# lucidrains/transfusion-pytorch

Measured on AMD Instinct MI355X. Metric: train samples/sec, dim512 d8 seq1024 text+latent, higher is better.
Workload: dtype bf16; 1 GPU; BASELINE config 2: Transfusion dim=512 depth=8 heads=8 dim_head=64 num_text_tokens=256 dim_latent=384; per-GPU batch 64 x seq 1024 (32 x [24 text tokens + (4,384) latent] per sample); step = pack + fwd + bwd + clip(0.5) + Adam(3e-4) (one GPU: no gradient exchange); global_batch=64, seq_len=1024, parallelism=dp1

## Files before the change

transfusion_pytorch_amd/csrc/attention.hip:

```cpp
#include "tfx_kernels.h"
#include "attn_asm_clobbers.inc"

namespace tfx {

constexpr int DH = 64;
constexpr int LDT = 72;

struct TileRegs { u32x4 r[2]; };
TFX_DEV void tile_gload(TileRegs& tr, const bf16* base, int ld, int row0, int nrows) {
#pragma unroll
  for (int i = 0; i < 2; i++) {
    int c = threadIdx.x + 256 * i;
    int row = min(row0 + (c >> 3), nrows - 1);
    tr.r[i] = *(const u32x4*)(base + (size_t)row * ld + (c & 7) * 8);
  }
}
TFX_DEV void tile_sstore(const TileRegs& tr, bf16* lds) {
#pragma unroll
  for (int i = 0; i < 2; i++) {
    int c = threadIdx.x + 256 * i;
    *(u32x4*)(lds + (c >> 3) * LDT + (c & 7) * 8) = tr.r[i];
  }
}
TFX_DEV bf16x8 lds_rowfrag(const bf16* lds, int r0, int ks) {
// ... 121 lines not shown
    int m = row_valid ? kve : 0;
#pragma unroll
    for (int o = 32; o > 0; o >>= 1) m = max(m, __shfl_xor(m, o, 64));
    if ((threadIdx.x & 63) == 0) kvl[threadIdx.x >> 6] = m;
    __syncthreads();
    lim = max(max(kvl[0], kvl[1]), max(kvl[2], kvl[3]));
  }
  return __builtin_amdgcn_readfirstlane(lim);
}
TFX_DEV bf16x8 pack8(const f32x16& v, int tt) {
  bf16x8 o;
#pragma unroll
  for (int e = 0; e < 8; e++) o[e] = f2bf(v[tt * 8 + e]);
  return o;
}
#define MFMA(a, b, c) __builtin_amdgcn_mfma_f32_32x32x16_bf16(a, b, c, 0, 0, 0)

TFX_DEV void wave_block_store(bf16* st, const bf16x4 (&v)[2][4], bf16* g0, int ld, int rows_valid, int lane = -1) {
  const int l = (lane >= 0 ? lane : (int)threadIdx.x) & 63, hi = l >> 5, r = l & 31, ch = l & 7;
  if (((ld & 7) | (int)(((uintptr_t)g0 >> 1) & 7)) != 0) {
    if (r < rows_valid) {
#pragma unroll
      for (int db = 0; db < 2; db++)
#pragma unroll
        for (int rg = 0; rg < 4; rg++) *(bf16x4*)(g0 + (size_t)r * ld + db * 32 + 8 * rg + 4 * hi) = v[db][rg];
    }
    return;
  }
#pragma unroll
  for (int db = 0; db < 2; db++)
#pragma unroll
    for (int rg = 0; rg < 4; rg++) {
      const int col = db * 32 + 8 * rg + 4 * hi;
      *(bf16x4*)(st + r * 64 + (((col >> 3) ^ ((r >> 1) & 7)) << 3) + (col & 7)) = v[db][rg];
    }
  bf16x8 t[4];
#pragma unroll
  for (int q = 0; q < 4; q++) {
    const int row = q * 8 + (l >> 3);
    t[q] = *(const bf16x8*)(st + row * 64 + ((ch ^ ((row >> 1) & 7)) << 3));
  }
#pragma unroll
  for (int q = 0; q < 4; q++) {
    const int row = q * 8 + (l >> 3);
    if (row < rows_valid) *(bf16x8*)(g0 + (size_t)row * ld + ch * 8) = t[q];
  }
}

template <int WHICH>
TFX_DEV void wave_block_store_nr(bf16* st, const bf16x4 (&v)[2][4], const tfx_attn_args& p, size_t tok, int colq, int rows_valid, float (&pg)[8], int lane = -1) {
  const int l = (lane >= 0 ? lane : (int)threadIdx.x) & 63, hi = l >> 5, r = l & 31, ch = l & 7;
  if (rows_valid <= 0) return;
#pragma unroll
  for (int db = 0; db < 2; db++)
#pragma unroll
    for (int rg = 0; rg < 4; rg++) {
      const int col = db * 32 + 8 * rg + 4 * hi;
      *(bf16x4*)(st + r * 64 + (((col >> 3) ^ ((r >> 1) & 7)) << 3) + (col & 7)) = v[db][rg];
    }
  if (!p.nr_gamma_q) {
    const int last = max(rows_valid - 1, 0);
    int pos[4];
#pragma unroll
    for (int q = 0; q < 4; q++) pos[q] = p.nr_rot_pos[tok + min(q * 8 + (l >> 3), last)];
#pragma unroll
    for (int q = 0; q < 4; q++) {
      const int row = q * 8 + (l >> 3), rd = min(row, last);
      const f32x4 cs = *(const f32x4*)(p.nr_cos + (size_t)pos[q] * 32 + ch * 4), sn = *(const f32x4*)(p.nr_sin + (size_t)pos[q] * 32 + ch * 4);
      const bf16x8 t = *(const bf16x8*)(st + rd * 64 + ((ch ^ ((rd >> 1) & 7)) << 3));
      const bf16x8 o = qk_rope_bwd_chunk(t, WHICH == 0 ? p.nr_q_scale : 1.f, cs, sn);
      if (row < rows_valid) *(bf16x8*)(p.nr_dqkv + (tok + row) * p.nr_ld_dqkv + colq + ch * 8) = o;
    }
    return;
  }
  const float sc = (WHICH == 0 ? p.nr_q_scale : 1.f) * (p.nr_norm_scale > 0.f ? p.nr_norm_scale : 8.f);
  const float* gmp = (WHICH == 0 ? p.nr_gamma_q : p.nr_gamma_k) + ch * 8;
  const f32x4 g0 = *(const f32x4*)gmp, g1 = *(const f32x4*)(gmp + 4);
  bf16x8 x8[4], t[4];
  f32x4 cs[4], sn[4];
  const int last = max(rows_valid - 1, 0);
#pragma unroll
  for (int q = 0; q < 4; q++) {
    const int row = min(q * 8 + (l >> 3), last);
    const size_t tt = tok + row;
    x8[q] = *(const bf16x8*)(p.nr_qkv + tt * p.nr_ld_qkv + colq + ch * 8);
    const int pos = p.nr_rot_pos[tt];
    cs[q] = *(const f32x4*)(p.nr_cos + (size_t)pos * 32 + ch * 4);
    sn[q] = *(const f32x4*)(p.nr_sin + (size_t)pos * 32 + ch * 4);
  }
#pragma unroll
  for (int q = 0; q < 4; q++) {
    const int row = min(q * 8 + (l >> 3), last);
    t[q] = *(const bf16x8*)(st + row * 64 + ((ch ^ ((row >> 1) & 7)) << 3));
  }
#pragma unroll
  for (int q = 0; q < 4; q++) {
    const int row = q * 8 + (l >> 3);
    const bool live = row < rows_valid;
    float xv[8], qq = 0.f;
#pragma unroll
    for (int e = 0; e < 8; e++) { xv[e] = bf2f(x8[q][e]); qq = fmaf(xv[e], xv[e], qq); }
    qq = group8_sum(qq);
    const float inv = qq > 1e-24f ? __builtin_amdgcn_rsqf(qq) : 1e12f;
    const float isc = live ? inv * sc : 0.f;
    float dyn[8], S = 0.f;
#pragma unroll
    for (int i = 0; i < 4; i++) {
      const float da = bf2f(t[q][2 * i]), db = bf2f(t[q][2 * i + 1]);
      const float ga = fmaf(db, sn[q][i], da * cs[q][i]);
      const float gb = fmaf(-da, sn[q][i], db * cs[q][i]);
      const float gma = i < 2 ? g0[2 * i] : g1[2 * i - 4], gmb = i < 2 ? g0[2 * i + 1] : g1[2 * i - 3];
      const float ca = sc * (1.f + gma), cb = sc * (1.f + gmb);
      const float ta = ga * xv[2 * i], tb = gb * xv[2 * i + 1];
      pg[2 * i] = fmaf(ta, isc, pg[2 * i]); pg[2 * i + 1] = fmaf(tb, isc, pg[2 * i + 1]);
      S = fmaf(ta, ca, S); S = fmaf(tb, cb, S);
      dyn[2 * i] = ga * ca; dyn[2 * i + 1] = gb * cb;
    }
    S = group8_sum(S);
    const float k = S * inv * inv * inv;
    bf16x8 o;
#pragma unroll
    for (int e = 0; e < 8; e++) o[e] = f2bf(fmaf(dyn[e], inv, -(xv[e] * k)));
    if (live) *(bf16x8*)(p.nr_dqkv + (tok + row) * p.nr_ld_dqkv + colq + ch * 8) = o;
  }
}
TFX_DEV void nr_flush_dgamma(float (&pg)[8], float* sg , float* dgamma, int t = -1) {
  const int tx = t >= 0 ? t : (int)threadIdx.x;
#pragma unroll
  for (int e = 0; e < 8; e++) {
#pragma unroll
    for (int m = 8; m < 64; m <<= 1) pg[e] += __shfl_xor(pg[e], m, 64);
  }
  const int lane = tx & 63, wv = tx >> 6;
  if (lane < 8) {
#pragma unroll
    for (int e = 0; e < 8; e++) sg[wv * 64 + lane * 8 + e] = pg[e];
  }
  __syncthreads();
  if (tx < 64) {
    const float s4 = sg[tx] + sg[64 + tx] + sg[128 + tx] + sg[192 + tx];
    if (s4 != 0.f) atomicAdd(dgamma + tx, s4);
  }
}
struct BlockId { int tile, h, b; };
TFX_DEV BlockId decode_block(int order, int ntile, bool heavy_last_tile) {
  BlockId o;
  (void)order;
  o.tile = heavy_last_tile ? ntile - 1 - (int)blockIdx.z : (int)blockIdx.z;
  o.h = blockIdx.x; o.b = blockIdx.y;
  return o;
}

#define MFMA_ACC(acc, a, b) asm volatile("v_mfma_f32_32x32x16_bf16 %0, %1, %2, %0" : "+v"(acc), "+v"(a), "+v"(b))
TFX_DEV void fwd_phase(const f32x16& s_cur, f32x16& s_nxt, u32x4 (&p_prev)[2], u32x4 (&p_cur)[2], f32x16 (&o)[2], const bf16x8 (&qf)[4],
                       const bf16* Kt_nxt, int kb_nxt, const bf16* Vt_prev, int kb_prev, float (&lsum)[2]) {
  const int hi = (threadIdx.x >> 5) & 1;
  bf16x8 frag[2];
  auto fetch = [&](int m) -> bf16x8 {
    if (m < 4) return dma_rowfrag(Kt_nxt, kb_nxt * 32, m);
    const int ra = kb_prev * 32 + 16 * ((m - 4) >> 1) + 4 * hi;
    return dma_tr8(Vt_prev, ra, ra + 8, (m & 1) * 32);
  };
  frag[0] = fetch(0);
#pragma unroll
  for (int ch = 0; ch < 8; ch++) {
    if (ch < 7) frag[(ch + 1) & 1] = fetch(ch + 1);
    float e0 = __builtin_amdgcn_exp2f(s_cur[2 * ch]), e1 = __builtin_amdgcn_exp2f(s_cur[2 * ch + 1]);
    if (ch == 0) asm volatile("v_mfma_f32_32x32x16_bf16 %0, %3, %4, 0" : "=&v"(s_nxt), "+v"(e0), "+v"(e1), "+v"(frag[0]) : "v"(qf[0]));
    else if (ch < 4) asm volatile("v_mfma_f32_32x32x16_bf16 %0, %3, %4, %0" : "+v"(s_nxt), "+v"(e0), "+v"(e1), "+v"(frag[ch & 1]) : "v"(qf[ch]));
    else asm volatile("v_mfma_f32_32x32x16_bf16 %0, %3, %4, %0" : "+v"(o[ch & 1]), "+v"(e0), "+v"(e1), "+v"(frag[ch & 1]), "+v"(p_prev[(ch - 4) >> 1]));
    lsum[0] += e0; lsum[1] += e1;
    bf16x2 pk2; pk2[0] = f2bf(e0); pk2[1] = f2bf(e1);
    uint32_t pk = __builtin_bit_cast(uint32_t, pk2);
    asm volatile("" : "+v"(lsum[0]), "+v"(lsum[1]), "+v"(pk));
    p_cur[ch >> 2][ch & 3] = pk;
    __builtin_amdgcn_sched_barrier(0);
  }
}

template <bool ROW>
TFX_DEV void fwd_phase_any(f32x16& s_cur, f32x16& s_nxt, u32x4 (&p_prev)[2], u32x4 (&p_cur)[2], f32x16 (&o)[2], const bf16x8 (&qf)[4],
                           const bf16* Kt_nxt, int kb_nxt, const bf16* Vt_prev, int kb_prev, float (&lsum)[2], const SoftCap& c, int key0, int kve,
                           bool mask, unsigned long long* ts = nullptr) {
#ifdef TFX_ATTN_TIMING
  unsigned long long t0 = __builtin_readcyclecounter();
#endif
  softcap16<ROW>(s_cur, c);
  if (mask) {
#pragma unroll
    for (int r = 0; r < 16; r++) s_cur[r] = key0 + (r & 3) + 8 * (r >> 2) < kve ? s_cur[r] : -__builtin_inff();
  }
#ifdef TFX_ATTN_TIMING
  asm volatile("" : "+v"(s_cur));
  unsigned long long t1 = __builtin_readcyclecounter();
#endif
  fwd_phase(s_cur, s_nxt, p_prev, p_cur, o, qf, Kt_nxt, kb_nxt, Vt_prev, kb_prev, lsum);
#ifdef TFX_ATTN_TIMING
  asm volatile("" : "+v"(s_nxt), "+v"(o[0]), "+v"(o[1]));
  ts[2] += t1 - t0; ts[3] += __builtin_readcyclecounter() - t1;
#endif
}

TFX_DEV void fwd_drain(u32x4 (&p_prev)[2], f32x16 (&o)[2], const bf16* Vt_prev, int kb_prev) {
  const int hi = (threadIdx.x >> 5) & 1;
  bf16x8 vt[4];
#pragma unroll
  for (int m = 0; m < 4; m++) { const int ra = kb_prev * 32 + 16 * (m >> 1) + 4 * hi; vt[m] = dma_tr8(Vt_prev, ra, ra + 8, (m & 1) * 32); }
#pragma unroll
  for (int m = 0; m < 4; m++) MFMA_ACC(o[m & 1], vt[m], p_prev[m >> 1]);
  asm volatile("s_nop 7" : "+v"(vt[0]), "+v"(vt[1]), "+v"(vt[2]), "+v"(vt[3]), "+v"(p_prev[0]), "+v"(p_prev[1]));
}

template <bool ASM, bool ROW = false>
__global__ __launch_bounds__(256, 2) void attn_fwd_pipe_kernel(tfx_attn_args p) {
  __shared__ __attribute__((aligned(1024))) bf16 Ks[3][64 * 64];
  __shared__ __attribute__((aligned(1024))) bf16 Vs[3][64 * 64];
  const int l = threadIdx.x & 63, w = threadIdx.x >> 6, hi = l >> 5;
  const BlockId bi = decode_block(p.order, (p.n + 127) / 128, true);
  const int h = bi.h, b = bi.b, q0 = bi.tile * 128;
  const int n = p.q_cnt ? p.q_cnt[b] : p.n;
  if (q0 >= n) return;
  const int nkv = p.n_kv > 0 ? p.n_kv : n;
  const size_t tok0 = p.q_row0 ? (size_t)p.q_row0[b] : (size_t)b * n, tokk = (size_t)b * nkv;
  const bf16* qb = p.q + tok0 * p.ld_q + h * DH;
  const bf16* kb_ = p.k + tokk * p.ld_k + h * DH;
  const bf16* vb = p.v + tokk * p.ld_v + h * DH;
  const int qrow = q0 + w * 32 + (l & 31);
  const int qc = min(qrow, n - 1);
  const int kve = p.kv_end[tok0 + qc];
  const int kv_limit = tile_kv_limit(p, tok0, q0, n, kve, qrow < n);
  const int nt = (kv_limit + 63) / 64;
  bf16x8 qf[4];
#pragma unroll
  for (int ks = 0; ks < 4; ks++) qf[ks] = g_rowfrag(qb, p.ld_q, qrow, n, ks);
  const SoftCap sc_ = make_softcap(p.softcap, p.sc_plan);
  const int kve_min = wave_min_i(kve);
  asm volatile("" : "+v"(qf[0]), "+v"(qf[1]), "+v"(qf[2]), "+v"(qf[3]));
  asm volatile("s_waitcnt vmcnt(0)" ::: "memory");
  tile_dma(kb_, p.ld_k, 0, nkv, Ks[0]);
  tile_dma(vb, p.ld_v, 0, nkv, Vs[0]);
  if (nt > 1) tile_dma(kb_, p.ld_k, 64, nkv, Ks[1]);

  f32x16 o[2], sA, sB;
  u32x4 pA[2], pB[2];
#pragma unroll
  for (int i = 0; i < 2; i++) {
#pragma unroll
    for (int r = 0; r < 16; r++) o[i][r] = 0.f;
#pragma unroll
    for (int e = 0; e < 4; e++) { pA[i][e] = 0u; pB[i][e] = 0u; }
  }
#pragma unroll
  for (int r = 0; r < 16; r++) { sA[r] = 0.f; sB[r] = 0.f; }
  float lsum[2] = {0.f, 0.f};
  int kslot = 0, vslot = 0;
#ifdef TFX_ATTN_TIMING
  unsigned long long tsec[4] = {0, 0, 0, 0}, tprev = __builtin_readcyclecounter();
#define AT_MARK(i) { const unsigned long long tn = __builtin_readcyclecounter(); tsec[i] += tn - tprev; tprev = tn; }
#define TS_ARG , tsec
#else
#define AT_MARK(i)
#define TS_ARG
#endif
  int j0 = 0;
  if constexpr (ASM) {
    const int kve_blk = __builtin_amdgcn_readfirstlane(p.kv_end[tok0 + q0]);
    const int nfull = __builtin_amdgcn_readfirstlane(min(kve_blk >> 6, (nkv - 128) >> 6));
    if (nfull > 0 && sc_.mode <= 1) {
      const int wu = __builtin_amdgcn_readfirstlane(w);
      const uint32_t ldsK = (uint32_t)(size_t)(lds_void_t*)&Ks[0][0], ldsV = (uint32_t)(size_t)(lds_void_t*)&Vs[0][0];
      uint32_t ka[4], vaA[2], vaB[2], dk[2], dv[2];
#pragma unroll
      for (int ks = 0; ks < 4; ks++) ka[ks] = ldsK + 2u * (uint32_t)((l & 31) * 64 + (((2 * ks + hi) ^ swz_f(l & 31)) << 3));
      {
        const int q = l & 15, ra = 4 * hi + (q >> 2), rb = ra + 8;
#pragma unroll
        for (int db = 0; db < 2; db++) {
          const int col = db * 32 + 16 * ((l >> 4) & 1) + 4 * (q & 3);
          vaA[db] = ldsV + 2u * (uint32_t)(ra * 64 + (((col >> 3) ^ swz_f(ra)) << 3) + (col & 7));
          vaB[db] = ldsV + 2u * (uint32_t)(rb * 64 + (((col >> 3) ^ swz_f(rb)) << 3) + (col & 7));
        }
      }
#pragma unroll
      for (int jp = 0; jp < 2; jp++) {
        const int r = w * 16 + jp * 8 + (l >> 3), c = (l & 7) ^ swz_f(r);
        dk[jp] = 2u * (uint32_t)(r * p.ld_k + c * 8);
        dv[jp] = 2u * (uint32_t)(r * p.ld_v + c * 8);
      }
      const uint64_t baseK = (uint64_t)(uintptr_t)kb_, baseV = (uint64_t)(uintptr_t)vb;
      u32x4 rsK, rsV;
      rsK[0] = __builtin_amdgcn_readfirstlane((uint32_t)baseK); rsK[1] = __builtin_amdgcn_readfirstlane((uint32_t)(baseK >> 32) & 0xffffu); rsK[2] = 0xffffff00u; rsK[3] = 0x00020000u;
      rsV[0] = __builtin_amdgcn_readfirstlane((uint32_t)baseV); rsV[1] = __builtin_amdgcn_readfirstlane((uint32_t)(baseV >> 32) & 0xffffu); rsV[2] = 0xffffff00u; rsV[3] = 0x00020000u;
      const uint32_t stk = __builtin_amdgcn_readfirstlane(128u * (uint32_t)p.ld_k), stv = __builtin_amdgcn_readfirstlane(128u * (uint32_t)p.ld_v);
      uint32_t sko = 2u * stk, svo = stv, cnt = (uint32_t)nfull;
      const uint32_t mk = __builtin_amdgcn_readfirstlane(ldsK + (uint32_t)wu * 2048u), mv = __builtin_amdgcn_readfirstlane(ldsV + (uint32_t)wu * 2048u);
      const float p1 = sc_.p1, p3 = sc_.p3, p5 = sc_.p5;
      u32x4 q0f = __builtin_bit_cast(u32x4, qf[0]), q1f = __builtin_bit_cast(u32x4, qf[1]), q2f = __builtin_bit_cast(u32x4, qf[2]), q3f = __builtin_bit_cast(u32x4, qf[3]);
#define AF_OPERANDS                                                                                                                                  \
          : [o0] "+&v"(o[0]), [o1] "+&v"(o[1]), "+{v[64:79]}"(sA), "+{v[104:107]}"(pB[0]), "+{v[108:111]}"(pB[1]), "+{v112}"(lsum[0]), "+{v113}"(lsum[1]),    \
            [sko] "+&s"(sko), [svo] "+&s"(svo), [cnt] "+&s"(cnt)                                                                                     \
          : [qf0] "v"(q0f), [qf1] "v"(q1f), [qf2] "v"(q2f), [qf3] "v"(q3f), [ka0] "v"(ka[0]), [ka1] "v"(ka[1]), [ka2] "v"(ka[2]), [ka3] "v"(ka[3]),  \
            [va0] "v"(vaA[0]), [va1] "v"(vaA[1]), [vb0] "v"(vaB[0]), [vb1] "v"(vaB[1]), [dk0] "v"(dk[0]), [dk1] "v"(dk[1]), [dv0] "v"(dv[0]), [dv1] "v"(dv[1]), \
            [rsk] "s"(rsK), [rsv] "s"(rsV), [stk] "s"(stk), [stv] "s"(stv), [mk] "s"(mk), [mv] "s"(mv), [p1] "v"(p1), [p3] AF_P3(p3), [p5] "s"(p5)   \
          : "memory", "scc", "v80", "v81", "v82", "v83", "v84", "v85", "v86", "v87", "v88", "v89", "v90", "v91", "v92", "v93", "v94", "v95",         \
            "v96", "v97", "v98", "v99", "v100", "v101", "v102", "v103", "v116", "v117", "v118", "v119", "v120", "v121", "v122", "v123", "v124",      \
            "v125", "v126", "v127", "v128", "v129", "v130", "v131", "v132", "v133", "v134", "v135", "v136", "v137", "v138", "v139", "v140", "v141",  \
            "v142", "v143", "v144", "v145", "v146", "v147", "v148", "v149", "v150", "v151"
      if (sc_.mode == 0) {
#define AF_P3 "s"
        asm volatile(
#include "attn_fwd_loop_m0.inc"
            AF_OPERANDS);
#undef AF_P3
      } else {
#define AF_P3 "v"
        asm volatile(
#include "attn_fwd_loop_m1.inc"
            AF_OPERANDS);
#undef AF_P3
      }
#undef AF_OPERANDS
      j0 = nfull;
      kslot = vslot = nfull % 3;
    }
  }
  for (int j = j0; j < nt; j++) {
    asm volatile("s_waitcnt vmcnt(0)" ::: "memory");
    __builtin_amdgcn_s_barrier();
    AT_MARK(0)
    const int kslot1 = kslot == 2 ? 0 : kslot + 1, kslot2 = kslot1 == 2 ? 0 : kslot1 + 1;
    const int vslot1 = vslot == 2 ? 0 : vslot + 1, vprev = vslot == 0 ? 2 : vslot - 1;
    if (j + 2 < nt) tile_dma(kb_, p.ld_k, (j + 2) * 64, nkv, Ks[kslot2]);
    if (j + 1 < nt) tile_dma(vb, p.ld_v, (j + 1) * 64, nkv, Vs[vslot1]);
    AT_MARK(1)
    if (j == 0) {
      sA = __builtin_amdgcn_mfma_f32_32x32x16_bf16(dma_rowfrag(Ks[0], 0, 0), qf[0], f32x16{}, 0, 0, 0);
#pragma unroll
      for (int ks = 1; ks < 4; ks++) sA = MFMA(dma_rowfrag(Ks[0], 0, ks), qf[ks], sA);
    }
    int u = 2 * j;
    fwd_phase_any<ROW>(sA, sB, pB, pA, o, qf, Ks[kslot], 1, j == 0 ? Vs[vslot] : Vs[vprev], 1, lsum, sc_, u * 32 + 4 * hi, kve, (u + 1) * 32 > kve_min TS_ARG);
    u = 2 * j + 1;
    fwd_phase_any<ROW>(sB, sA, pA, pB, o, qf, Ks[kslot1], 0, Vs[vslot], 0, lsum, sc_, u * 32 + 4 * hi, kve, (u + 1) * 32 > kve_min TS_ARG);
    kslot = kslot1; vslot = vslot1;
#ifdef TFX_ATTN_TIMING
    tprev = __builtin_readcyclecounter();
#endif
  }
#ifdef TFX_ATTN_TIMING
  if (l == 0) {
    unsigned long long* ob = (unsigned long long*)p.dq + ((((size_t)b * p.h + h) * ((n + 127) / 128) + bi.tile) * 4 + w) * 5;
    for (int i = 0; i < 4; i++) ob[i] = tsec[i];
    ob[4] = nt;
  }
#endif
#undef AT_MARK
#undef TS_ARG
  fwd_drain(pB, o, Vs[vslot == 0 ? 2 : vslot - 1], 1);
  asm volatile("s_nop 15\n\ts_nop 15" : "+v"(o[0]), "+v"(o[1]));
  float ls = lsum[0] + lsum[1];
  ls += __shfl_xor(ls, 32, 64);
  {
    const float g = p.gate ? sigmoidf_(bf2f(p.gate[(tok0 + qc) * p.ld_gate + h])) : 1.f;
    bf16x4 ov[2][4];
    if (p.laser) {
      const float rl = __builtin_amdgcn_rcpf(ls);
#pragma unroll
      for (int db = 0; db < 2; db++)
#pragma unroll
        for (int rg = 0; rg < 4; rg++)
#pragma unroll
          for (int e = 0; e < 4; e++) ov[db][rg][e] = f2bf(g * __logf(o[db][rg * 4 + e] * rl));
    } else {
      const float sc = g * __builtin_amdgcn_rcpf(ls);
#pragma unroll
      for (int db = 0; db < 2; db++)
#pragma unroll
        for (int rg = 0; rg < 4; rg++)
#pragma unroll
          for (int e = 0; e < 4; e++) ov[db][rg][e] = f2bf(o[db][rg * 4 + e] * sc);
    }
    __syncthreads();
    wave_block_store(&Ks[0][0] + w * 2048, ov, p.out + (tok0 + q0 + w * 32) * p.ld_out + h * DH, p.ld_out, n - (q0 + w * 32));
    if (qrow < n && hi == 0) p.lse[((size_t)b * p.h + h) * p.n + qrow] = __log2f(ls) * LN2;
  }
}

__global__ __launch_bounds__(256) void attn_bwd_prep_kernel(tfx_attn_args p) {
  const unsigned gid = blockIdx.x * blockDim.x + threadIdx.x;
  const unsigned vid = gid >> 3;
  const int sub = gid & 7;
  const unsigned T = (unsigned)p.b * p.n;
  if (vid >= T * p.h) return;
  const unsigned t = vid / (unsigned)p.h; const int h = (int)(vid - t * p.h);
  const bf16x8 d8 = *(const bf16x8*)(p.dout + (size_t)t * p.ld_dout + h * DH + sub * 8);
  const bf16x8 o8 = *(const bf16x8*)(p.out + (size_t)t * p.ld_out + h * DH + sub * 8);
  const float g = p.gate ? sigmoidf_(bf2f(p.gate[(size_t)t * p.ld_gate + h])) : 1.f;
  if (p.laser) {
    const float rg = __builtin_amdgcn_rcpf(fmaxf(g, 1e-30f));
    float dg = 0.f, ds = 0.f; bf16x8 e8;
#pragma unroll
    for (int e = 0; e < 8; e++) {
      const float d = bf2f(d8[e]), og = bf2f(o8[e]);
      dg += d * og; ds += d;
      e8[e] = f2bf(d * g * __expf(-og * rg));
    }
    *(bf16x8*)(p.do_eff + (size_t)t * p.ld_do + h * DH + sub * 8) = e8;
    dg = group8_sum(dg); ds = group8_sum(ds);
    if (sub == 0) {
      const unsigned bb = t / (unsigned)p.n, i = t - bb * p.n;
      p.delta[((size_t)bb * p.h + h) * p.n + i] = ds * g;
      if (p.gate) p.dgate[(size_t)t * p.ld_dgate + h] = f2bf(dg * (1.f - g));
    }
    return;
  }
  float dl = 0.f; bf16x8 e8;
#pragma unroll
  for (int e = 0; e < 8; e++) { float d = bf2f(d8[e]); dl += d * bf2f(o8[e]); e8[e] = f2bf(d * g); }
  *(bf16x8*)(p.do_eff + (size_t)t * p.ld_do + h * DH + sub * 8) = e8;
  dl = group8_sum(dl);
  if (sub == 0) {
    const unsigned bb = t / (unsigned)p.n, i = t - bb * p.n;
    p.delta[((size_t)bb * p.h + h) * p.n + i] = dl;
    if (p.gate) p.dgate[(size_t)t * p.ld_dgate + h] = f2bf(dl * (1.f - g));
  }
}

__global__ __launch_bounds__(256, 2) void attn_bwd_dq_kernel(tfx_attn_args p) {
  __shared__ __attribute__((aligned(16))) bf16 Ks[64 * LDT];
  __shared__ __attribute__((aligned(16))) bf16 Vs[64 * LDT];
  const int l = threadIdx.x & 63, w = threadIdx.x >> 6, hi = l >> 5;
  const int n = p.n;
  const BlockId bi = decode_block(p.order, (n + 127) / 128, true);
  const int h = bi.h, b = bi.b, q0 = bi.tile * 128;
  const size_t tok0 = (size_t)b * n;
  const bf16* qb = p.q + tok0 * p.ld_q + h * DH;
  const bf16* kb_ = p.k + tok0 * p.ld_k + h * DH;
  const bf16* vb = p.v + tok0 * p.ld_v + h * DH;
  const bf16* dob = p.do_eff + tok0 * p.ld_do + h * DH;
  const int qrow = q0 + w * 32 + (l & 31);
  const int qc = min(qrow, n - 1);
  const int kve = p.kv_end[tok0 + qc];
  const int kv_limit = p.kv_end[tok0 + min(q0 + 127, n - 1)];
  const int nt = (kv_limit + 63) / 64;
  const float lse2 = p.lse[((size_t)b * p.h + h) * n + qc] * LOG2E;
  float dlt;
  const int kve_min = wave_min_i(kve);

  bf16x8 qf[4], dof[4];
  dlt = p.delta[((size_t)b * p.h + h) * n + qc];
#pragma unroll
  for (int ks = 0; ks < 4; ks++) { qf[ks] = g_rowfrag(qb, p.ld_q, qrow, n, ks); dof[ks] = g_rowfrag(dob, p.ld_do, qrow, n, ks); }
  f32x16 dq[2];
#pragma unroll
  for (int i = 0; i < 2; i++)
#pragma unroll
    for (int r = 0; r < 16; r++) dq[i][r] = 0.f;
  const SoftCap sc_ = make_softcap(p.softcap, p.sc_plan);
  f32x16 zero16;
#pragma unroll
  for (int r = 0; r < 16; r++) zero16[r] = 0.f;
  asm volatile("" : "+v"(zero16));

  TileRegs kr, vr;
  tile_gload(kr, kb_, p.ld_k, 0, n);
  tile_gload(vr, vb, p.ld_v, 0, n);
  for (int j = 0; j < nt; j++) {
    __syncthreads();
    tile_sstore(kr, Ks); tile_sstore(vr, Vs);
    __syncthreads();
    if (j + 1 < nt) { tile_gload(kr, kb_, p.ld_k, (j + 1) * 64, n); tile_gload(vr, vb, p.ld_v, (j + 1) * 64, n); }
    const bool need_mask = (j + 1) * 64 > kve_min;
#pragma unroll
    for (int kb = 0; kb < 2; kb++) {
      f32x16 s = MFMA(lds_rowfrag(Ks, kb * 32, 0), qf[0], zero16);
      f32x16 dp = MFMA(lds_rowfrag(Vs, kb * 32, 0), dof[0], zero16);
#pragma unroll
      for (int ks = 1; ks < 4; ks++) {
        s = MFMA(lds_rowfrag(Ks, kb * 32, ks), qf[ks], s);
        dp = MFMA(lds_rowfrag(Vs, kb * 32, ks), dof[ks], dp);
      }
      if (sc_.mode == 0) {
#pragma unroll
        for (int r = 0; r < 16; r++) {
          const float u = s[r] * s[r];
          dp[r] = (dp[r] - dlt) * fmaf(u, sc_.d3, sc_.d1);
          s[r] = __builtin_amdgcn_exp2f(fmaf(s[r], fmaf(u, sc_.p3, sc_.p1), -lse2));
        }
      } else if (sc_.mode == 1) {
#pragma unroll
        for (int r = 0; r < 16; r++) {
          const float u = s[r] * s[r];
          dp[r] = (dp[r] - dlt) * fmaf(u, fmaf(u, sc_.d5, sc_.d3), sc_.d1);
          s[r] = __builtin_amdgcn_exp2f(fmaf(s[r], fmaf(u, fmaf(u, sc_.p5, sc_.p3), sc_.p1), -lse2));
        }
      } else {
        softcap16(s, sc_);
#pragma unroll
        for (int r = 0; r < 16; r++) {
          const float dth = fmaf(s[r] * s[r], -sc_.g2, 1.f);
          dp[r] = (dp[r] - dlt) * dth;
          s[r] = __builtin_amdgcn_exp2f(s[r] - lse2);
        }
      }
      if (need_mask) {
        const int key0 = j * 64 + kb * 32 + 4 * hi;
#pragma unroll
        for (int r = 0; r < 16; r++) s[r] = key0 + (r & 3) + 8 * (r >> 2) < kve ? s[r] : 0.f;
      }
#pragma unroll
      for (int r = 0; r < 16; r++) s[r] *= dp[r];
#pragma unroll
      for (int tt = 0; tt < 2; tt++) {
        const bf16x8 dsf = pack8(s, tt);
        const int ra = kb * 32 + 16 * tt + 4 * hi;
#pragma unroll
        for (int db = 0; db < 2; db++) dq[db] = MFMA(lds_tr8(Ks, LDT, ra, ra + 8, db * 32), dsf, dq[db]);
      }
    }
  }
  {
    bf16x4 ov[2][4];
#pragma unroll
    for (int db = 0; db < 2; db++)
#pragma unroll
      for (int rg = 0; rg < 4; rg++)
#pragma unroll
        for (int e = 0; e < 4; e++) ov[db][rg][e] = f2bf(dq[db][rg * 4 + e]);
    __syncthreads();
    if (p.nr_qkv) {
      __shared__ float sg[4 * 64];
      float pg[8];
#pragma unroll
      for (int e = 0; e < 8; e++) pg[e] = 0.f;
      wave_block_store_nr<0>((w < 2 ? Ks : Vs) + (w & 1) * 2048, ov, p, tok0 + q0 + w * 32, h * DH, n - (q0 + w * 32), pg);
      if (p.nr_gamma_q) nr_flush_dgamma(pg, sg, p.nr_dgamma_q);
    } else
    wave_block_store((w < 2 ? Ks : Vs) + (w & 1) * 2048, ov, p.dq + (tok0 + q0 + w * 32) * p.ld_dq + h * DH, p.ld_dq, n - (q0 + w * 32));
// ... 239 lines not shown
  for (int rg = 0; rg < 4; rg++) {
    const int ql = ql0 + 8 * rg;
    const f32x4 ls4 = *(const f32x4*)(s_lse + ql), dl4 = *(const f32x4*)(s_dlt + ql);
    const int* kv4 = s_kve + ql;
#pragma unroll
    for (int e = 0; e < 4; e++) {
      const int r = rg * 4 + e;
      const float a = s[r];
      float arg, dth;
      if constexpr (MODE == 0) {
        const float u = a * a;
        dth = fmaf(u, c.d3, c.d1);
        arg = fmaf(a, fmaf(u, c.p3, c.p1), -ls4[e]);
      } else if constexpr (MODE == 1) {
        const float u = a * a;
        dth = fmaf(u, fmaf(u, c.d5, c.d3), c.d1);
        arg = fmaf(a, fmaf(u, fmaf(u, c.p5, c.p3), c.p1), -ls4[e]);
      } else {
        dth = fmaf(a * a, -g2, 1.f);
        arg = a - ls4[e];
      }
      float pv = __builtin_amdgcn_exp2f(arg);
      if (MASK) pv = krow < kv4[e] ? pv : 0.f;
      pr[r] = pv;
      s[r] = pv * ((dp[r] - dl4[e]) * dth);
    }
  }
}

__global__ __launch_bounds__(256, 2) void attn_bwd_dkv_kernel(tfx_attn_args p) {
  __shared__ __attribute__((aligned(16))) bf16 Qs[64 * LDT];
  __shared__ __attribute__((aligned(16))) bf16 Ds[64 * LDT];
  __shared__ __attribute__((aligned(16))) float s_lse[64], s_dlt[64];
  __shared__ __attribute__((aligned(16))) int s_kve[64];
  const int l = threadIdx.x & 63, w = threadIdx.x >> 6, hi = l >> 5;
  const int n = p.n;
  const BlockId bi = decode_block(p.order, (n + 127) / 128, false);
  const int h = bi.h, b = bi.b, k0 = bi.tile * 128;
  const size_t tok0 = (size_t)b * n;
  const bf16* qb = p.q + tok0 * p.ld_q + h * DH;
  const bf16* kb_ = p.k + tok0 * p.ld_k + h * DH;
  const bf16* vb = p.v + tok0 * p.ld_v + h * DH;
  const bf16* dob = p.do_eff + tok0 * p.ld_do + h * DH;
  const float* lseb = p.lse + ((size_t)b * p.h + h) * n;
  const float* dltb = p.delta + ((size_t)b * p.h + h) * n;
  const int krow = k0 + w * 32 + (l & 31);
  const int qt0 = p.q_start[tok0 + min(k0, n - 1)] / 64;
  const int qt1 = (n + 63) / 64;

  bf16x8 kf[4], vf[4];
#pragma unroll
  for (int ks = 0; ks < 4; ks++) { kf[ks] = g_rowfrag(kb_, p.ld_k, krow, n, ks); vf[ks] = g_rowfrag(vb, p.ld_v, krow, n, ks); }
  f32x16 dk[2], dv[2];
#pragma unroll
  for (int i = 0; i < 2; i++)
#pragma unroll
    for (int r = 0; r < 16; r++) { dk[i][r] = 0.f; dv[i][r] = 0.f; }
  const SoftCap sc_ = make_softcap(p.softcap, p.sc_plan);
  const int kw_last = k0 + w * 32 + 31;

  TileRegs qr, dr;
  float st_l = 0.f, st_d = 0.f; int st_k = 0;
  auto stats_gload = [&](int jt) {
    if (threadIdx.x < 64) {
      const int qi = jt * 64 + threadIdx.x;
      const int qcl = min(qi, n - 1);
      st_l = lseb[qcl]; st_d = dltb[qcl];
      st_k = qi < n ? p.kv_end[tok0 + qcl] : 0;
    }
  };
  tile_gload(qr, qb, p.ld_q, qt0 * 64, n);
  tile_gload(dr, dob, p.ld_do, qt0 * 64, n);
  stats_gload(qt0);
  for (int jt = qt0; jt < qt1; jt++) {
    __syncthreads();
    tile_sstore(qr, Qs); tile_sstore(dr, Ds);
    if (threadIdx.x < 64) { s_lse[threadIdx.x] = st_l * LOG2E; s_dlt[threadIdx.x] = st_d; s_kve[threadIdx.x] = st_k; }
    __syncthreads();
    if (jt + 1 < qt1) { tile_gload(qr, qb, p.ld_q, (jt + 1) * 64, n); tile_gload(dr, dob, p.ld_do, (jt + 1) * 64, n); stats_gload(jt + 1); }
#pragma unroll
    for (int qb2 = 0; qb2 < 2; qb2++) {
      {
        const int lastr = min(31, n - 1 - (jt * 64 + qb2 * 32));
        if (__builtin_amdgcn_readfirstlane((int)(lastr < 0 || s_kve[qb2 * 32 + max(lastr, 0)] <= k0 + w * 32)) != 0) continue;
      }
      f32x16 s, dp;
#pragma unroll
      for (int r = 0; r < 16; r++) { s[r] = 0.f; dp[r] = 0.f; }
#pragma unroll
      for (int ks = 0; ks < 4; ks++) {
        s = MFMA(lds_rowfrag(Qs, qb2 * 32, ks), kf[ks], s);
        dp = MFMA(lds_rowfrag(Ds, qb2 * 32, ks), vf[ks], dp);
      }
      if (sc_.mode == 2) softcap16(s, sc_);
      const bool need_mask = __builtin_amdgcn_readfirstlane((int)(kw_last >= s_kve[qb2 * 32] || jt * 64 + qb2 * 32 + 31 >= n)) != 0;
      f32x16 pr;
      const int ql0 = qb2 * 32 + 4 * hi;
      if (sc_.mode == 0) {
        if (need_mask) dkv_scores<true, 0>(s, dp, pr, s_lse, s_dlt, s_kve, ql0, krow, sc_.g2, sc_);
        else dkv_scores<false, 0>(s, dp, pr, s_lse, s_dlt, s_kve, ql0, krow, sc_.g2, sc_);
      } else if (sc_.mode == 1) {
        if (need_mask) dkv_scores<true, 1>(s, dp, pr, s_lse, s_dlt, s_kve, ql0, krow, sc_.g2, sc_);
        else dkv_scores<false, 1>(s, dp, pr, s_lse, s_dlt, s_kve, ql0, krow, sc_.g2, sc_);
      } else {
        if (need_mask) dkv_scores<true, 2>(s, dp, pr, s_lse, s_dlt, s_kve, ql0, krow, sc_.g2, sc_);
        else dkv_scores<false, 2>(s, dp, pr, s_lse, s_dlt, s_kve, ql0, krow, sc_.g2, sc_);
      }
#pragma unroll
      for (int tt = 0; tt < 2; tt++) {
        const bf16x8 pf = pack8(pr, tt), dsf = pack8(s, tt);
        const int ra = qb2 * 32 + 16 * tt + 4 * hi;
#pragma unroll
        for (int db = 0; db < 2; db++) {
          dv[db] = MFMA(lds_tr8(Ds, LDT, ra, ra + 8, db * 32), pf, dv[db]);
          dk[db] = MFMA(lds_tr8(Qs, LDT, ra, ra + 8, db * 32), dsf, dk[db]);
        }
      }
    }
  }
  {
    bf16x4 kv[2][4], vv[2][4];
#pragma unroll
    for (int db = 0; db < 2; db++)
#pragma unroll
      for (int rg = 0; rg < 4; rg++)
#pragma unroll
        for (int e = 0; e < 4; e++) { kv[db][rg][e] = f2bf(dk[db][rg * 4 + e]); vv[db][rg][e] = f2bf(dv[db][rg * 4 + e]); }
    __syncthreads();
    bf16* st = (w < 2 ? Qs : Ds) + (w & 1) * 2048;
    const int rows = n - (k0 + w * 32);
    if (p.nr_qkv) {
      __shared__ float sg[4 * 64];
      float pg[8];
#pragma unroll
      for (int e = 0; e < 8; e++) pg[e] = 0.f;
      wave_block_store_nr<1>(st, kv, p, tok0 + k0 + w * 32, (p.h + h) * DH, rows, pg);
      wave_block_store(st, vv, p.dv + (tok0 + k0 + w * 32) * p.ld_dv + h * DH, p.ld_dv, rows);
      if (p.nr_gamma_q) nr_flush_dgamma(pg, sg, p.nr_dgamma_k);
    } else {
      wave_block_store(st, kv, p.dk + (tok0 + k0 + w * 32) * p.ld_dk + h * DH, p.ld_dk, rows);
      wave_block_store(st, vv, p.dv + (tok0 + k0 + w * 32) * p.ld_dv + h * DH, p.ld_dv, rows);
    }
  }
}

static dim3 attn_grid(const tfx_attn_args& q) { return dim3(q.h, q.b, (q.n + 127) / 128); }
int attn_fwd(const tfx_attn_args& p, hipStream_t s) {
  if (p.n <= 0 || p.b <= 0 || p.h <= 0) return -1;
  if ((p.ld_q | p.ld_k | p.ld_v | p.ld_out) & 7) return -2;
  if (!(p.softcap > 0.f) || p.softcap * LOG2E > 96.f) return -3;
  tfx_attn_args q = p; q.order = 1;
  static int use_asm = -1;
  if (use_asm < 0) { const char* e = getenv("TFX_ATTN_ASM"); use_asm = (e && e[0] == '1') ? 1 : 0; }
  if (use_asm && p.n_kv == 0 && !p.q_cnt && !p.q_row0 && p.sc_plan) hipLaunchKernelGGL(attn_fwd_pipe_kernel<true>, attn_grid(q), dim3(256), 0, s, q);
  else if (p.n_kv > 0 || p.q_cnt || p.q_row0) hipLaunchKernelGGL((attn_fwd_pipe_kernel<false, true>), attn_grid(q), dim3(256), 0, s, q);
  else hipLaunchKernelGGL(attn_fwd_pipe_kernel<false>, attn_grid(q), dim3(256), 0, s, q);
  return (int)hipGetLastError();
}
int attn_bwd(const tfx_attn_args& p, hipStream_t s) {
  if (p.n <= 0 || p.b <= 0 || p.h <= 0) return -1;
  if ((p.ld_q | p.ld_k | p.ld_v | p.ld_out | p.ld_dout | p.ld_do | p.ld_dq | p.ld_dk | p.ld_dv) & 7) return -2;
  if (!(p.softcap > 0.f) || p.softcap * LOG2E > 96.f) return -3;
  long long nthreads = (long long)p.b * p.n * p.h * 8;
  if (nthreads >= (1ll << 31)) return -4;
  if (p.nr_qkv) {
    if (!p.nr_dqkv || !p.nr_gamma_q != !p.nr_gamma_k || !p.nr_rot_pos || !p.nr_cos || !p.nr_sin) return -5;
    if (p.nr_gamma_q && (!p.nr_dgamma_q || !p.nr_dgamma_k)) return -5;
    if (((p.nr_ld_qkv | p.nr_ld_dqkv) & 7) || (((uintptr_t)p.nr_qkv | (uintptr_t)p.nr_dqkv) & 15)) return -5;
  }
  tfx_attn_args q = p; q.order = 1;
  static int pipe = -1;
  if (pipe < 0) { const char* e = getenv("TFX_ATTN_BWD_PIPE"); pipe = (e && e[0] == '0') ? 0 : 1; }
  hipLaunchKernelGGL(attn_bwd_prep_kernel, dim3((unsigned)((nthreads + 255) / 256)), dim3(256), 0, s, q);
  hipLaunchKernelGGL(attn_bwd_dkv_kernel, attn_grid(q), dim3(256), 0, s, q);
  if (pipe) hipLaunchKernelGGL(attn_bwd_dq_pipe_kernel, attn_grid(q), dim3(256), 0, s, q);
  else hipLaunchKernelGGL(attn_bwd_dq_kernel, attn_grid(q), dim3(256), 0, s, q);
  return (int)hipGetLastError();
}

}
```

Before: 2619 samples/s.

## Stop attention forward compute early per wave at its last needed key block

Adds a STOP variant of the forward attention kernel, on by default. Each wave computes the last 32-key chunk any of its rows can attend to and stops softmax/MFMA work there. For the remaining tiles it only takes part in barriers and DMA issue, so block-level synchronisation still holds. A half-tile tail path skips the next-S MFMAs, and a per-block hash rotates wave-to-row assignment to spread the imbalance. This cuts wasted masked work in the causal/latent-block attention pattern, at the cost of more code paths and possible correctness risk in the slot bookkeeping.

```diff
diff --git a/transfusion_pytorch_amd/csrc/attention.hip b/transfusion_pytorch_amd/csrc/attention.hip
--- a/transfusion_pytorch_amd/csrc/attention.hip
+++ b/transfusion_pytorch_amd/csrc/attention.hip
@@ -297,21 +297,26 @@
 }
 
 #define MFMA_ACC(acc, a, b) asm volatile("v_mfma_f32_32x32x16_bf16 %0, %1, %2, %0" : "+v"(acc), "+v"(a), "+v"(b))
+#ifdef TFX_ATTN_TIMING
+enum { AT_PROLOGUE = 4, AT_TILE_INT, AT_TILE_BND, AT_NTILE_INT, AT_NTILE_BND, AT_DRAIN, AT_EPI_BARRIER, AT_STORE_ISSUE, AT_STORE_ACK, AT_NT, AT_LU, AT_LIFE, AT_NSEC };
+#endif
+template <bool S_NXT = true>
 TFX_DEV void fwd_phase(const f32x16& s_cur, f32x16& s_nxt, u32x4 (&p_prev)[2], u32x4 (&p_cur)[2], f32x16 (&o)[2], const bf16x8 (&qf)[4],
-                       const bf16* Kt_nxt, int kb_nxt, const bf16* Vt_prev, int kb_prev, float (&lsum)[2]) {
-  const int hi = (threadIdx.x >> 5) & 1;
+                       const bf16* Kt_nxt, int kb_nxt, const bf16* Vt_prev, int kb_prev, float (&lsum)[2], int lane = -1) {
+  const int hi = ((lane >= 0 ? lane : (int)threadIdx.x) >> 5) & 1;
   bf16x8 frag[2];
   auto fetch = [&](int m) -> bf16x8 {
-    if (m < 4) return dma_rowfrag(Kt_nxt, kb_nxt * 32, m);
+    if (m < 4) return dma_rowfrag(Kt_nxt, kb_nxt * 32, m, lane);
     const int ra = kb_prev * 32 + 16 * ((m - 4) >> 1) + 4 * hi;
-    return dma_tr8(Vt_prev, ra, ra + 8, (m & 1) * 32);
+    return dma_tr8(Vt_prev, ra, ra + 8, (m & 1) * 32, lane);
   };
-  frag[0] = fetch(0);
+  if (S_NXT) frag[0] = fetch(0);
 #pragma unroll
   for (int ch = 0; ch < 8; ch++) {
-    if (ch < 7) frag[(ch + 1) & 1] = fetch(ch + 1);
+    if (ch < 7 && (S_NXT || ch >= 3)) frag[(ch + 1) & 1] = fetch(ch + 1);
     float e0 = __builtin_amdgcn_exp2f(s_cur[2 * ch]), e1 = __builtin_amdgcn_exp2f(s_cur[2 * ch + 1]);
-    if (ch == 0) asm volatile("v_mfma_f32_32x32x16_bf16 %0, %3, %4, 0" : "=&v"(s_nxt), "+v"(e0), "+v"(e1), "+v"(frag[0]) : "v"(qf[0]));
+    if (ch < 4 && !S_NXT) asm volatile("" : "+v"(e0), "+v"(e1));
+    else if (ch == 0) asm volatile("v_mfma_f32_32x32x16_bf16 %0, %3, %4, 0" : "=&v"(s_nxt), "+v"(e0), "+v"(e1), "+v"(frag[0]) : "v"(qf[0]));
     else if (ch < 4) asm volatile("v_mfma_f32_32x32x16_bf16 %0, %3, %4, %0" : "+v"(s_nxt), "+v"(e0), "+v"(e1), "+v"(frag[ch & 1]) : "v"(qf[ch]));
     else asm volatile("v_mfma_f32_32x32x16_bf16 %0, %3, %4, %0" : "+v"(o[ch & 1]), "+v"(e0), "+v"(e1), "+v"(frag[ch & 1]), "+v"(p_prev[(ch - 4) >> 1]));
     lsum[0] += e0; lsum[1] += e1;
@@ -323,10 +328,10 @@
   }
 }
 
-template <bool ROW>
+template <bool ROW, bool S_NXT = true>
 TFX_DEV void fwd_phase_any(f32x16& s_cur, f32x16& s_nxt, u32x4 (&p_prev)[2], u32x4 (&p_cur)[2], f32x16 (&o)[2], const bf16x8 (&qf)[4],
                            const bf16* Kt_nxt, int kb_nxt, const bf16* Vt_prev, int kb_prev, float (&lsum)[2], const SoftCap& c, int key0, int kve,
-                           bool mask, unsigned long long* ts = nullptr) {
+                           bool mask, unsigned long long* ts = nullptr, int lane = -1) {
 #ifdef TFX_ATTN_TIMING
   unsigned long long t0 = __builtin_readcyclecounter();
 #endif
@@ -339,30 +344,45 @@
   asm volatile("" : "+v"(s_cur));
   unsigned long long t1 = __builtin_readcyclecounter();
 #endif
-  fwd_phase(s_cur, s_nxt, p_prev, p_cur, o, qf, Kt_nxt, kb_nxt, Vt_prev, kb_prev, lsum);
+  fwd_phase<S_NXT>(s_cur, s_nxt, p_prev, p_cur, o, qf, Kt_nxt, kb_nxt, Vt_prev, kb_prev, lsum, lane);
 #ifdef TFX_ATTN_TIMING
   asm volatile("" : "+v"(s_nxt), "+v"(o[0]), "+v"(o[1]));
   ts[2] += t1 - t0; ts[3] += __builtin_readcyclecounter() - t1;
 #endif
 }
 
-TFX_DEV void fwd_drain(u32x4 (&p_prev)[2], f32x16 (&o)[2], const bf16* Vt_prev, int kb_prev) {
-  const int hi = (threadIdx.x >> 5) & 1;
+TFX_DEV void fwd_drain(u32x4 (&p_prev)[2], f32x16 (&o)[2], const bf16* Vt_prev, int kb_prev, int lane = -1) {
+  const int hi = ((lane >= 0 ? lane : (int)threadIdx.x) >> 5) & 1;
   bf16x8 vt[4];
 #pragma unroll
-  for (int m = 0; m < 4; m++) { const int ra = kb_prev * 32 + 16 * (m >> 1) + 4 * hi; vt[m] = dma_tr8(Vt_prev, ra, ra + 8, (m & 1) * 32); }
+  for (int m = 0; m < 4; m++) { const int ra = kb_prev * 32 + 16 * (m >> 1) + 4 * hi; vt[m] = dma_tr8(Vt_prev, ra, ra + 8, (m & 1) * 32, lane); }
 #pragma unroll
   for (int m = 0; m < 4; m++) MFMA_ACC(o[m & 1], vt[m], p_prev[m >> 1]);
   asm volatile("s_nop 7" : "+v"(vt[0]), "+v"(vt[1]), "+v"(vt[2]), "+v"(vt[3]), "+v"(p_prev[0]), "+v"(p_prev[1]));
 }
 
-template <bool ASM, bool ROW = false>
+template <bool ASM, bool ROW = false, bool STOP = false>
 __global__ __launch_bounds__(256, 2) void attn_fwd_pipe_kernel(tfx_attn_args p) {
   __shared__ __attribute__((aligned(1024))) bf16 Ks[3][64 * 64];
   __shared__ __attribute__((aligned(1024))) bf16 Vs[3][64 * 64];
-  const int l = threadIdx.x & 63, w = threadIdx.x >> 6, hi = l >> 5;
+#ifdef TFX_ATTN_TIMING
+  unsigned long long tsec[AT_NT], tprev = __builtin_readcyclecounter();
+  const unsigned long long tborn = tprev;
+#pragma unroll
+  for (int i = 0; i < AT_NT; i++) tsec[i] = 0;
+#define AT_MARK(i) { const unsigned long long tn = __builtin_readcyclecounter(); tsec[i] += tn - tprev; tprev = tn; }
+#define TS_ARG , tsec
+#define TS_ARG_L , tsec,
+#else
+#define AT_MARK(i)
+#define TS_ARG
+#define TS_ARG_L , nullptr,
+#endif
+  const int l = threadIdx.x & 63, hi = l >> 5;
   const BlockId bi = decode_block(p.order, (p.n + 127) / 128, true);
   const int h = bi.h, b = bi.b, q0 = bi.tile * 128;
+  const unsigned lin = blockIdx.x + gridDim.x * (blockIdx.y + gridDim.y * blockIdx.z);
+  const int w = STOP ? (int)((__builtin_amdgcn_readfirstlane(threadIdx.x >> 6) + (lin ^ (lin >> 2) ^ (lin >> 4) ^ (lin >> 6) ^ (lin >> 8) ^ (lin >> 10))) & 3) : (int)(threadIdx.x >> 6);
   const int n = p.q_cnt ? p.q_cnt[b] : p.n;
   if (q0 >= n) return;
   const int nkv = p.n_kv > 0 ? p.n_kv : n;
@@ -380,11 +400,13 @@
   for (int ks = 0; ks < 4; ks++) qf[ks] = g_rowfrag(qb, p.ld_q, qrow, n, ks);
   const SoftCap sc_ = make_softcap(p.softcap, p.sc_plan);
   const int kve_min = wave_min_i(kve);
+  const int lu = STOP ? min(max(wave_max_i(qrow < n ? kve : 0) - 1, 0) >> 5, 2 * nt - 1) : 2 * nt - 1;
   asm volatile("" : "+v"(qf[0]), "+v"(qf[1]), "+v"(qf[2]), "+v"(qf[3]));
   asm volatile("s_waitcnt vmcnt(0)" ::: "memory");
   tile_dma(kb_, p.ld_k, 0, nkv, Ks[0]);
   tile_dma(vb, p.ld_v, 0, nkv, Vs[0]);
   if (nt > 1) tile_dma(kb_, p.ld_k, 64, nkv, Ks[1]);
+  AT_MARK(AT_PROLOGUE)
 
   f32x16 o[2], sA, sB;
   u32x4 pA[2], pB[2];
@@ -399,14 +421,6 @@
   for (int r = 0; r < 16; r++) { sA[r] = 0.f; sB[r] = 0.f; }
   float lsum[2] = {0.f, 0.f};
   int kslot = 0, vslot = 0;
-#ifdef TFX_ATTN_TIMING
-  unsigned long long tsec[4] = {0, 0, 0, 0}, tprev = __builtin_readcyclecounter();
-#define AT_MARK(i) { const unsigned long long tn = __builtin_readcyclecounter(); tsec[i] += tn - tprev; tprev = tn; }
-#define TS_ARG , tsec
-#else
-#define AT_MARK(i)
-#define TS_ARG
-#endif
   int j0 = 0;
   if constexpr (ASM) {
     const int kve_blk = __builtin_amdgcn_readfirstlane(p.kv_end[tok0 + q0]);
@@ -469,39 +483,67 @@
       kslot = vslot = nfull % 3;
     }
   }
-  for (int j = j0; j < nt; j++) {
-    asm volatile("s_waitcnt vmcnt(0)" ::: "memory");
-    __builtin_amdgcn_s_barrier();
-    AT_MARK(0)
-    const int kslot1 = kslot == 2 ? 0 : kslot + 1, kslot2 = kslot1 == 2 ? 0 : kslot1 + 1;
-    const int vslot1 = vslot == 2 ? 0 : vslot + 1, vprev = vslot == 0 ? 2 : vslot - 1;
-    if (j + 2 < nt) tile_dma(kb_, p.ld_k, (j + 2) * 64, nkv, Ks[kslot2]);
-    if (j + 1 < nt) tile_dma(vb, p.ld_v, (j + 1) * 64, nkv, Vs[vslot1]);
-    AT_MARK(1)
-    if (j == 0) {
-      sA = __builtin_amdgcn_mfma_f32_32x32x16_bf16(dma_rowfrag(Ks[0], 0, 0), qf[0], f32x16{}, 0, 0, 0);
-#pragma unroll
-      for (int ks = 1; ks < 4; ks++) sA = MFMA(dma_rowfrag(Ks[0], 0, ks), qf[ks], sA);
-    }
+#ifdef TFX_ATTN_TIMING
+  unsigned long long ttile = tprev;
+#define AT_TILE_END(j) { const unsigned long long tn = __builtin_readcyclecounter(); const int bnd = (2 * (j) + 2) * 32 > kve_min ? 1 : 0;               \
+                         tsec[AT_TILE_INT + bnd] += tn - ttile; tsec[AT_NTILE_INT + bnd] += 1; ttile = tn; tprev = tn; }
+#else
+#define AT_TILE_END(j)
+#endif
+#define FWD_TILE_TOP(j)                                                                                                                                \
+    asm volatile("s_waitcnt vmcnt(0)" ::: "memory");                                            \
+    __builtin_amdgcn_s_barrier();                                              \
+    AT_MARK(0)                                                                                                                                         \
+    const int kslot1 = kslot == 2 ? 0 : kslot + 1, kslot2 = kslot1 == 2 ? 0 : kslot1 + 1;                                                             \
+    const int vslot1 = vslot == 2 ? 0 : vslot + 1, vprev = vslot == 0 ? 2 : vslot - 1;                                                                \
+    if ((j) + 2 < nt) tile_dma(kb_, p.ld_k, ((j) + 2) * 64, nkv, Ks[kslot2]);                                                                         \
+    if ((j) + 1 < nt) tile_dma(vb, p.ld_v, ((j) + 1) * 64, nkv, Vs[vslot1]);                                                                          \
+    AT_MARK(1)                                                                                                                                         \
+    if ((j) == 0) {                                                                                                   \
+      sA = __builtin_amdgcn_mfma_f32_32x32x16_bf16(dma_rowfrag(Ks[0], 0, 0), qf[0], f32x16{}, 0, 0, 0);                                               \
+      _Pragma("unroll") for (int ks = 1; ks < 4; ks++) sA = MFMA(dma_rowfrag(Ks[0], 0, ks), qf[ks], sA);                                              \
+    }
+  const int jf = STOP ? (lu + 1) >> 1 : nt;
+  int j = j0;
+  for (; j < jf; j++) {
+    FWD_TILE_TOP(j)
     int u = 2 * j;
     fwd_phase_any<ROW>(sA, sB, pB, pA, o, qf, Ks[kslot], 1, j == 0 ? Vs[vslot] : Vs[vprev], 1, lsum, sc_, u * 32 + 4 * hi, kve, (u + 1) * 32 > kve_min TS_ARG);
     u = 2 * j + 1;
     fwd_phase_any<ROW>(sB, sA, pA, pB, o, qf, Ks[kslot1], 0, Vs[vslot], 0, lsum, sc_, u * 32 + 4 * hi, kve, (u + 1) * 32 > kve_min TS_ARG);
     kslot = kslot1; vslot = vslot1;
-#ifdef TFX_ATTN_TIMING
-    tprev = __builtin_readcyclecounter();
-#endif
-  }
-#ifdef TFX_ATTN_TIMING
-  if (l == 0) {
-    unsigned long long* ob = (unsigned long long*)p.dq + ((((size_t)b * p.h + h) * ((n + 127) / 128) + bi.tile) * 4 + w) * 5;
-    for (int i = 0; i < 4; i++) ob[i] = tsec[i];
-    ob[4] = nt;
-  }
-#endif
-#undef AT_MARK
-#undef TS_ARG
-  fwd_drain(pB, o, Vs[vslot == 0 ? 2 : vslot - 1], 1);
+    AT_TILE_END(j)
+  }
+  if (STOP && !(lu & 1)) {
+    FWD_TILE_TOP(j)
+    const int tl = -1;
+    fwd_phase_any<ROW, false>(sA, sB, pB, pA, o, qf, Ks[kslot], 1, j == 0 ? Vs[vslot] : Vs[vprev], 1, lsum, sc_, lu * 32 + 4 * hi, kve, (lu + 1) * 32 > kve_min TS_ARG_L tl);
+#pragma unroll
+    for (int i = 0; i < 2; i++) pB[i] = pA[i];
+    kslot = kslot1; vslot = vslot1;
+    AT_TILE_END(j)
+    j++;
+  }
+  {
+    int tl = threadIdx.x & 63;
+    asm volatile("" : "+v"(tl));
+    fwd_drain(pB, o, Vs[vslot == 0 ? 2 : vslot - 1], STOP ? lu & 1 : 1, tl);
+  }
+  if constexpr (STOP) {
+    for (; j < nt; j++) {
+      asm volatile("s_waitcnt vmcnt(0)" ::: "memory");
+      __builtin_amdgcn_s_barrier();
+      AT_MARK(0)
+      const int kslot1 = kslot == 2 ? 0 : kslot + 1, kslot2 = kslot1 == 2 ? 0 : kslot1 + 1, vslot1 = vslot == 2 ? 0 : vslot + 1;
+      if (j + 2 < nt) tile_dma(kb_, p.ld_k, (j + 2) * 64, nkv, Ks[kslot2]);
+      if (j + 1 < nt) tile_dma(vb, p.ld_v, (j + 1) * 64, nkv, Vs[vslot1]);
+      AT_MARK(1)
+      kslot = kslot1; vslot = vslot1;
+      AT_TILE_END(j)
+    }
+  }
+#undef FWD_TILE_TOP
+#undef AT_TILE_END
   asm volatile("s_nop 15\n\ts_nop 15" : "+v"(o[0]), "+v"(o[1]));
   float ls = lsum[0] + lsum[1];
   ls += __shfl_xor(ls, 32, 64);
@@ -525,10 +567,28 @@
 #pragma unroll
           for (int e = 0; e < 4; e++) ov[db][rg][e] = f2bf(o[db][rg * 4 + e] * sc);
     }
+#ifdef TFX_ATTN_TIMING
+    asm volatile("" : "+v"(ov[0][0]), "+v"(ov[1][3]));
+#endif
+    AT_MARK(AT_DRAIN)
     __syncthreads();
+    AT_MARK(AT_EPI_BARRIER)
     wave_block_store(&Ks[0][0] + w * 2048, ov, p.out + (tok0 + q0 + w * 32) * p.ld_out + h * DH, p.ld_out, n - (q0 + w * 32));
     if (qrow < n && hi == 0) p.lse[((size_t)b * p.h + h) * p.n + qrow] = __log2f(ls) * LN2;
-  }
+#ifdef TFX_ATTN_TIMING
+    AT_MARK(AT_STORE_ISSUE)
+    asm volatile("s_waitcnt vmcnt(0)" ::: "memory");
+    AT_MARK(AT_STORE_ACK)
+    if (l == 0 && p.dq) {
+      unsigned long long* ob = (unsigned long long*)p.dq + ((((size_t)b * p.h + h) * ((n + 127) / 128) + bi.tile) * 4 + w) * AT_NSEC;
+      for (int i = 0; i < AT_NT; i++) ob[i] = tsec[i];
+      ob[AT_NT] = nt; ob[AT_LU] = lu; ob[AT_LIFE] = tprev - tborn;
+    }
+#endif
+  }
+#undef AT_MARK
+#undef TS_ARG
+#undef TS_ARG_L
 }
 
 __global__ __launch_bounds__(256) void attn_bwd_prep_kernel(tfx_attn_args p) {
@@ -1074,9 +1134,14 @@
   tfx_attn_args q = p; q.order = 1;
   static int use_asm = -1;
   if (use_asm < 0) { const char* e = getenv("TFX_ATTN_ASM"); use_asm = (e && e[0] == '1') ? 1 : 0; }
-  if (use_asm && p.n_kv == 0 && !p.q_cnt && !p.q_row0 && p.sc_plan) hipLaunchKernelGGL(attn_fwd_pipe_kernel<true>, attn_grid(q), dim3(256), 0, s, q);
-  else if (p.n_kv > 0 || p.q_cnt || p.q_row0) hipLaunchKernelGGL((attn_fwd_pipe_kernel<false, true>), attn_grid(q), dim3(256), 0, s, q);
-  else hipLaunchKernelGGL(attn_fwd_pipe_kernel<false>, attn_grid(q), dim3(256), 0, s, q);
+  static int stop = -1;
+  if (stop < 0) { const char* e = getenv("TFX_ATTN_FWD_STOP"); stop = (e && e[0] == '0') ? 0 : 1; }
+  const bool row = p.n_kv > 0 || p.q_cnt || p.q_row0;
+  if (use_asm && !row && p.sc_plan) hipLaunchKernelGGL(attn_fwd_pipe_kernel<true>, attn_grid(q), dim3(256), 0, s, q);
+  else if (row && stop) hipLaunchKernelGGL((attn_fwd_pipe_kernel<false, true, true>), attn_grid(q), dim3(256), 0, s, q);
+  else if (row) hipLaunchKernelGGL((attn_fwd_pipe_kernel<false, true, false>), attn_grid(q), dim3(256), 0, s, q);
+  else if (stop) hipLaunchKernelGGL((attn_fwd_pipe_kernel<false, false, true>), attn_grid(q), dim3(256), 0, s, q);
+  else hipLaunchKernelGGL((attn_fwd_pipe_kernel<false, false, false>), attn_grid(q), dim3(256), 0, s, q);
   return (int)hipGetLastError();
 }
 int attn_bwd(const tfx_attn_args& p, hipStream_t s) {
```

New measurement: 2621 samples/s (median of 4 runs). Within noise of the previous version (+0.1%).
